# techshoww/RoMa

Hardware: AMD Instinct MI355X
Metric: image-pairs/sec at 560->864 (higher is better)
Workload: dtype fp16; 1 GPU; roma_outdoor 560->864 full coarse-to-fine symmetric match (BASELINE configs[1]; configs[2] = --pairs 8 --gpus 8); launch=eager launches, coarse_res=560, upsample_res=864, parallelism=single GPU

## Files before the change

include/roma_hip.h:

```cpp
#ifndef ROMA_HIP_H
#define ROMA_HIP_H

#include <stdint.h>

#ifdef __cplusplus
extern "C" {
#endif

#define ROMA_ABI_VERSION 5

enum { ROMA_F32 = 0, ROMA_F16 = 1, ROMA_BF16 = 2 };
enum { ROMA_NCHW = 0, ROMA_NHWC = 1 };
enum { ROMA_LC_AUTO = 0, ROMA_LC_TILE8X4 = 1, ROMA_LC_TILE8X8 = 2, ROMA_LC_ROWS8 = 3 };
enum { ROMA_E_ARG = -1, ROMA_E_DTYPE = -2, ROMA_E_SHAPE = -3, ROMA_E_ALIGN = -4, ROMA_E_UNSUPPORTED = -5 };

int roma_abi_version(void);
const char* roma_last_error(void);

int roma_local_corr(const void* f0, const void* f1, const float* flow, void* out,
                    int B, int C, int H, int W, int r, int dtype,
                    int layout, int f0_pitch, int f1_pitch, int out_layout, int out_pitch, int f1_batch_shift, int variant,
                    void* stream);

int roma_warp_bilinear(const void* src, const float* flow, void* dst,
// ... 13 lines not shown
                          void* stream);

int roma_flow_update(float* flow, float* cert, const float* cert_in, const float* delta,
                     int B, int H, int W, float sx, float sy, void* stream);

int roma_cls_to_flow_refine(const void* logits, float* flow_out, float* cert_out,
                            int B, int C, int HW, long stride_b, long stride_c, long stride_p,
                            int dtype, void* stream);

int roma_cos_kernel(const void* x, const void* y, float* K, int B, int N, int M, int D, int dtype, int x_pitch, int y_pitch,
                    int y_batch_shift, float T, float eps, float diag_add, void* stream);

int roma_chol_diag_block(float* A, int lda, long strideA, float* W, int ldw, long strideW, int nb, int B, int* info,
                         int info_base, void* stream);

int roma_chol_step(float* A, int lda, long strideA, int n, int ncols, int j, int nb, const float* W, int ldw, long strideW, float* R,
                   int ldr, long strideR, float* Wn, int ldwn, long strideWn, int* info, int info_base, int B, void* stream);

int roma_chol_subst_step(int dir, const float* W, int ldw, long strideW, const float* R, long strideRb, long strideRs, int ldr, float* T,
                         long strideTb, long strideTs, int ldt, int t_in_panel, float* X, int ldx, long strideX, int n, int m, int nb,
                         int s, int B, void* stream);

int roma_attention_fwd(const void* q, const void* k, const void* v, void* o, int B, int H, int Nq, int Nk, int head_dim, long q_sb,
                       long q_sn, long q_sh, long k_sb, long k_sn, long k_sh, long v_sb, long v_sn, long v_sh, long o_sb, long o_sn,
                       long o_sh, float scale, int dtype, void* stream);

int roma_match_finalize(const float* flow, const float* cert, const float* cert16, float* warp, float* certainty,
                        int P, int H, int W, int H16, int W16, int symmetric, void* stream);

int roma_kde_density(const float* x, float* density, int N, int down, float std, int half_mode, void* stream);

int roma_race_keys(const float* p, const long* counter, float* keys, long N, float thresh, unsigned seed, unsigned stage,
                   void* stream);

long roma_race_select_workspace(int P, long N, int k);
int roma_race_select(const float* p, const long* counter, const long* seeds, int P, long N, int k, float thresh, unsigned stage,
                     long* sel_key, long* sel_idx, void* workspace, long workspace_bytes, void* stream);

int roma_kde_density_batch(const float* x, const long* index, float* density, int P, long N, int n, int down, float std,
                           int half_mode, void* stream);

int roma_nn_argmin(const float* q, const float* r, int* idx, int NQ, int NR, void* stream);

int roma_resample_u8(const void* in, void* out, int H, int W, int C, int out_size, int axis, const int* bounds,
                     const int* coef, int ksize, void* stream);
int roma_normalize_u8(const void* in, float* out, int H, int W, const float* mean3, const float* std3, void* stream);

int roma_bias_relu_nchw(void* x, const void* bias, int B, int C, int HW, int dtype, void* stream);

int roma_bias_relu_pool2_nchw(void* x, const void* bias, void* pooled, int B, int C, int H, int W, int dtype, void* stream);

int roma_bias_relu_nhwc(void* x, const void* bias, long npix, int C, int dtype, void* stream);
int roma_bias_relu_pool2_nhwc(void* x, const void* bias, void* pooled, int B, int C, int H, int W, int dtype, void* stream);

int roma_dwconv5x5_bn_relu(const void* x, const float* w, const float* scale, const float* shift, void* y,
                           int B, int C, int H, int W, int dtype, int x_pitch, int y_pitch, void* stream);

int roma_refiner_block(const void* x, const void* w25, const float* scale, const float* shift, const void* wt,
                       const float* bias, void* y, int B, int C, int H, int W, int kpad, int dtype, int x_pitch, int y_pitch,
                       void* stream);

int roma_refiner_wide_pack(const void* wt, void* wp, int D);
int roma_refiner_wide_taps(const void* w25, void* w25p, int D);
int roma_refiner_block_wide(const void* x, const void* w25p, const float* scale, const float* shift, const void* wp,
                            const float* bias, void* y, int B, int H, int W, int D, int x_pitch, int y_pitch, int dtype,
                            void* stream);

int roma_pointwise_mfma(const void* x, const void* wt, const float* bias, void* y, long M, int C, int kpad, int dtype,
                        int x_pitch, int y_pitch, void* stream);

int roma_refiner_block_mid(const void* x, const float* w25, const float* scale, const float* shift, const void* wt,
                           const float* bias, void* y, int B, int C, int H, int W, int dtype, int x_pitch, int y_pitch,
                           void* stream);

int roma_refiner_head(const void* x, const float* wo, const float* bo, float* flow, const float* cert_in, float* cert_out,
                      float* delta_out, int B, int H, int W, int C, int pitch, int dtype, float sx, float sy, void* stream);

int roma_pointwise_small(const void* x, const float* wt, const float* bias, void* y, long M, int C, int dtype,
                         int x_pitch, int y_pitch, void* stream);

int roma_project_skinny(const void* x, const void* wt, const float* bias, void* y, long M, int K, int N, int dtype, int x_pitch,
                        int y_pitch, void* stream);

int roma_add_layernorm(void* x, int x_dtype, long x_stride, const void* y, int y_dtype, long y_stride, const float* ls,
                       const float* gamma, const float* beta, void* out, int out_dtype, long out_stride, long rows, int C,
                       float eps, void* stream);

int roma_tiny_corr_posembed(const float* f0, const float* f1, float* out, int B, int C,
                            int H0, int W0, int H1, int W1, int exact, void* stream);

int roma_jpeg_info(const void* data, long nbytes, int* info);
int roma_jpeg_entropy_decode(const void* data, long nbytes, int16_t* coef, uint16_t* qt);
int roma_jpeg_reconstruct(const int16_t* coef, const uint16_t* qt, void* planes, void* rgb, const int* info, void* stream);

long roma_ransac_workspace(int kind, int P, int N, int iters, long* offsets);
int roma_ransac_hypotheses(int kind, const double* xa, const double* xb, int P, int N, int iters, float threshold, unsigned seed,
                           int p0, void* ws, long ws_bytes, void* stream);
int roma_ransac_select(int kind, const double* xa, const double* xb, int P, int N, int iters, float threshold, int lo_iters,
                       const void* ws, long ws_bytes, double* model, unsigned char* mask, void* stream);

int roma_ransac_hypotheses_ex(int kind, const double* xa, const double* xb, int P, int N, int iters, float threshold, int scoring,
                              unsigned seed, int p0, void* ws, long ws_bytes, void* stream);
int roma_ransac_select_ex(int kind, const double* xa, const double* xb, int P, int N, int iters, float threshold, int scoring,
                          int lo_iters, const void* ws, long ws_bytes, double* model, unsigned char* mask, void* stream);
int roma_magsac_table(float* loss, float* weight);

// ... 60 lines not shown
```

roma_amd/_lib.py:

```python
from __future__ import annotations

import ctypes
import os
from ctypes import c_char_p, c_float, c_int, c_long, c_void_p

_HERE = os.path.dirname(os.path.abspath(__file__))
LIB_PATH = os.path.join(_HERE, "csrc", "libroma_hip.so")

ROMA_F32, ROMA_F16, ROMA_BF16 = 0, 1, 2
ROMA_NCHW, ROMA_NHWC = 0, 1
LC_VARIANTS = {"auto": 0, "tile8x4": 1, "tile8x8": 2, "rows8": 3}
ABI_VERSION = 5
SCORE_MSAC, SCORE_MAGSAC = 0, 1
ROMA_E_ARG, ROMA_E_DTYPE, ROMA_E_SHAPE, ROMA_E_ALIGN, ROMA_E_UNSUPPORTED = -1, -2, -3, -4, -5

SIGNATURES = {
    "roma_abi_version": [],
    "roma_last_error": [],
    "roma_local_corr": [c_void_p, c_void_p, c_void_p, c_void_p, c_int, c_int, c_int, c_int, c_int, c_int,
                        c_int, c_int, c_int, c_int, c_int, c_int, c_int, c_void_p],
    "roma_warp_bilinear": [c_void_p, c_void_p, c_void_p, c_int, c_int, c_int, c_int, c_int, c_int, c_int,
                           c_int, c_int, c_int, c_int, c_int, c_void_p],
    "roma_disp_emb": [c_void_p, c_void_p, c_void_p, c_void_p, c_int, c_int, c_int, c_int, c_float, c_int, c_int, c_int, c_void_p],
    "roma_interp_bilinear": [c_void_p, c_void_p, c_int, c_int, c_int, c_int, c_int, c_void_p],
    "roma_interp_bilinear_pair": [c_void_p, c_void_p, c_int, c_void_p, c_void_p, c_int, c_int, c_int, c_int, c_int, c_void_p],
    "roma_refiner_assemble": [c_void_p, c_void_p, c_void_p, c_void_p, c_void_p, c_int, c_int, c_int, c_int, c_int, c_int, c_int, c_int,
                              c_int, c_int, c_int, c_float, c_int, c_void_p],
    "roma_project_skinny": [c_void_p, c_void_p, c_void_p, c_void_p, c_long, c_int, c_int, c_int, c_int, c_int, c_void_p],
    "roma_flow_update": [c_void_p, c_void_p, c_void_p, c_void_p, c_int, c_int, c_int, c_float, c_float, c_void_p],
    "roma_cls_to_flow_refine": [c_void_p, c_void_p, c_void_p, c_int, c_int, c_int, c_long, c_long, c_long, c_int, c_void_p],
    "roma_cos_kernel": [c_void_p, c_void_p, c_void_p, c_int, c_int, c_int, c_int, c_int, c_int, c_int, c_int, c_float, c_float,
                        c_float, c_void_p],
    "roma_add_layernorm": [c_void_p, c_int, c_long, c_void_p, c_int, c_long, c_void_p, c_void_p, c_void_p, c_void_p, c_int, c_long,
                           c_long, c_int, c_float, c_void_p],
    "roma_attention_fwd": [c_void_p, c_void_p, c_void_p, c_void_p, c_int, c_int, c_int, c_int, c_int] + [c_long] * 12 + [c_float, c_int, c_void_p],
    "roma_chol_diag_block": [c_void_p, c_int, c_long, c_void_p, c_int, c_long, c_int, c_int, c_void_p, c_int, c_void_p],
    "roma_chol_step": [c_void_p, c_int, c_long, c_int, c_int, c_int, c_int, c_void_p, c_int, c_long, c_void_p, c_int, c_long,
                       c_void_p, c_int, c_long, c_void_p, c_int, c_int, c_void_p],
    "roma_chol_subst_step": [c_int, c_void_p, c_int, c_long, c_void_p, c_long, c_long, c_int, c_void_p, c_long, c_long, c_int, c_int,
                             c_void_p, c_int, c_long, c_int, c_int, c_int, c_int, c_int, c_void_p],
    "roma_match_finalize": [c_void_p, c_void_p, c_void_p, c_void_p, c_void_p, c_int, c_int, c_int, c_int, c_int, c_int, c_void_p],
    "roma_kde_density": [c_void_p, c_void_p, c_int, c_int, c_float, c_int, c_void_p],
    "roma_nn_argmin": [c_void_p, c_void_p, c_void_p, c_int, c_int, c_void_p],
    "roma_race_keys": [c_void_p, c_void_p, c_void_p, c_long, c_float, ctypes.c_uint, ctypes.c_uint, c_void_p],
    "roma_race_select_workspace": [c_int, c_long, c_int],
    "roma_race_select": [c_void_p, c_void_p, c_void_p, c_int, c_long, c_int, c_float, ctypes.c_uint, c_void_p, c_void_p, c_void_p, c_long,
                         c_void_p],
    "roma_kde_density_batch": [c_void_p, c_void_p, c_void_p, c_int, c_long, c_int, c_int, c_float, c_int, c_void_p],
    "roma_dwconv5x5_bn_relu": [c_void_p, c_void_p, c_void_p, c_void_p, c_void_p, c_int, c_int, c_int, c_int, c_int, c_int, c_int, c_void_p],
    "roma_resample_u8": [c_void_p, c_void_p, c_int, c_int, c_int, c_int, c_int, c_void_p, c_void_p, c_int, c_void_p],
    "roma_normalize_u8": [c_void_p, c_void_p, c_int, c_int, c_void_p, c_void_p, c_void_p],
    "roma_bias_relu_nchw": [c_void_p, c_void_p, c_int, c_int, c_int, c_int, c_void_p],
    "roma_bias_relu_pool2_nchw": [c_void_p, c_void_p, c_void_p, c_int, c_int, c_int, c_int, c_int, c_void_p],
    "roma_bias_relu_nhwc": [c_void_p, c_void_p, c_long, c_int, c_int, c_void_p],
    "roma_bias_relu_pool2_nhwc": [c_void_p, c_void_p, c_void_p, c_int, c_int, c_int, c_int, c_int, c_void_p],
    "roma_pointwise_mfma": [c_void_p, c_void_p, c_void_p, c_void_p, c_long, c_int, c_int, c_int, c_int, c_int, c_void_p],
    "roma_refiner_block": [c_void_p, c_void_p, c_void_p, c_void_p, c_void_p, c_void_p, c_void_p, c_int, c_int, c_int, c_int, c_int, c_int,
                           c_int, c_int, c_void_p],
    "roma_refiner_block_mid": [c_void_p, c_void_p, c_void_p, c_void_p, c_void_p, c_void_p, c_void_p, c_int, c_int, c_int, c_int, c_int, c_int,
                               c_int, c_void_p],
    "roma_refiner_wide_pack": [c_void_p, c_void_p, c_int],
    "roma_refiner_wide_taps": [c_void_p, c_void_p, c_int],
    "roma_jpeg_info": [c_void_p, c_long, c_void_p],
    "roma_jpeg_entropy_decode": [c_void_p, c_long, c_void_p, c_void_p],
    "roma_jpeg_reconstruct": [c_void_p, c_void_p, c_void_p, c_void_p, c_void_p, c_void_p],
    "roma_refiner_block_wide": [c_void_p, c_void_p, c_void_p, c_void_p, c_void_p, c_void_p, c_void_p, c_int, c_int, c_int, c_int, c_int, c_int,
                                c_int, c_void_p],
    "roma_refiner_head": [c_void_p, c_void_p, c_void_p, c_void_p, c_void_p, c_void_p, c_void_p, c_int, c_int, c_int, c_int, c_int, c_int,
                          c_float, c_float, c_void_p],
    "roma_pointwise_small": [c_void_p, c_void_p, c_void_p, c_void_p, c_long, c_int, c_int, c_int, c_int, c_void_p],
    "roma_tiny_corr_posembed": [c_void_p, c_void_p, c_void_p, c_int, c_int, c_int, c_int, c_int, c_int, c_int, c_void_p],
    "roma_ransac_workspace": [c_int, c_int, c_int, c_int, c_void_p],
    "roma_ransac_hypotheses": [c_int, c_void_p, c_void_p, c_int, c_int, c_int, c_float, ctypes.c_uint, c_int, c_void_p, c_long, c_void_p],
    "roma_ransac_select": [c_int, c_void_p, c_void_p, c_int, c_int, c_int, c_float, c_int, c_void_p, c_long, c_void_p, c_void_p,
                           c_void_p],
    "roma_ransac_hypotheses_ex": [c_int, c_void_p, c_void_p, c_int, c_int, c_int, c_float, c_int, ctypes.c_uint, c_int, c_void_p, c_long,
                                  c_void_p],
    "roma_ransac_select_ex": [c_int, c_void_p, c_void_p, c_int, c_int, c_int, c_float, c_int, c_int, c_void_p, c_long, c_void_p, c_void_p,
                              c_void_p],
    "roma_magsac_table": [c_void_p, c_void_p],
    "roma_essential_workspace": [c_int, c_int, c_int, c_void_p],
    "roma_essential_hypotheses": [c_void_p, c_void_p, c_void_p, c_void_p, c_int, c_int, c_int, c_float, ctypes.c_uint, c_int, c_void_p,
                                  c_long, c_void_p],
    "roma_essential_select": [c_void_p, c_void_p, c_void_p, c_void_p, c_int, c_int, c_int, c_float, c_int, c_void_p, c_long, c_void_p,
                              c_void_p, c_void_p],
    "roma_essential_hypotheses_ex": [c_void_p, c_void_p, c_void_p, c_void_p, c_int, c_int, c_int, c_float, c_int, ctypes.c_uint, c_int,
                                     c_void_p, c_long, c_void_p],
    "roma_essential_select_ex": [c_void_p, c_void_p, c_void_p, c_void_p, c_int, c_int, c_int, c_float, c_int, c_int, c_void_p, c_long,
                                 c_void_p, c_void_p, c_void_p],
    "roma_recover_pose": [c_void_p, c_void_p, c_void_p, c_void_p, c_void_p, c_void_p, c_int, c_int, c_void_p, c_void_p, c_void_p,
                          c_void_p, c_void_p],
    "roma_refine_pose": [c_void_p, c_void_p, c_void_p, c_void_p, c_void_p, c_void_p, c_void_p, c_int, c_int, ctypes.c_double, c_int,
                         c_void_p, c_void_p, c_void_p, c_void_p, c_void_p, c_void_p, c_void_p],
    "roma_refine_fundamental": [c_void_p, c_void_p, c_void_p, c_void_p, c_int, c_int, ctypes.c_double, c_int, c_void_p, c_void_p, c_void_p,
                                c_void_p, c_void_p, c_void_p],
    "roma_refine_homography": [c_void_p, c_void_p, c_void_p, c_void_p, c_int, c_int, ctypes.c_double, c_int, c_void_p, c_void_p, c_void_p,
                               c_void_p, c_void_p, c_void_p],
    "roma_triangulate": [c_void_p, c_void_p, c_void_p, c_void_p, c_void_p, c_void_p, c_void_p, c_int, c_int, c_int, c_float, c_float,
                         c_void_p, c_void_p, c_void_p, c_void_p, c_void_p, c_void_p, c_void_p],
    "roma_triangulate_nview": [c_void_p, c_void_p, c_void_p, c_long, c_void_p, c_void_p, c_void_p, c_int, c_int, c_int, c_long, c_long,
                               c_float, c_int, c_int, c_int, c_float, c_float, c_void_p, c_void_p, c_void_p, c_void_p, c_void_p, c_void_p,
                               c_void_p],
    "roma_warp_kpts": [c_void_p, c_int, c_void_p, c_void_p, c_void_p, c_void_p, c_void_p, c_int, c_int, c_int, c_int, c_int, c_int, c_int,
                       ctypes.c_double, c_void_p, c_void_p, c_void_p, c_void_p],
    "roma_dense_match_metrics": [c_void_p, c_long, c_void_p, c_void_p, c_void_p, c_void_p, c_void_p, c_int, c_int, c_int, c_int, c_int, c_int,
                                 c_int, c_int, ctypes.c_double, c_void_p, c_long, c_void_p, c_void_p, c_void_p, c_void_p, c_void_p],
    "roma_absolute_pose_workspace": [c_int, c_int, c_int, c_void_p],
    "roma_absolute_pose_hypotheses": [c_void_p, c_void_p, c_void_p, c_int, c_int, c_int, c_float, c_int, ctypes.c_uint, c_int, c_void_p,
# ... 42 lines not shown
```

roma_amd/csrc/bias_relu.hip:

```cpp
#include "common.h"

namespace roma {
namespace {

template <typename T, int VEC>
__global__ __launch_bounds__(256) void bias_relu_kernel(T* __restrict__ x, const T* __restrict__ bias, int C, int HW) {
  const int plane = blockIdx.y;
  const float bv = to_f32(bias[plane % C]);
  T* p = x + (size_t)plane * HW;
  const int nvec = HW / VEC;
  for (int i = blockIdx.x * 256 + threadIdx.x; i < nvec; i += gridDim.x * 256) {
    if constexpr (VEC == 8) {
      u32x4 v = reinterpret_cast<u32x4*>(p)[i];
      float f[8];
      unpack16<T>(v, f);
#pragma unroll
      for (int e = 0; e < 8; ++e) f[e] = fmaxf(f[e] + bv, 0.f);
      reinterpret_cast<u32x4*>(p)[i] = pack16<T>(f);
    } else {
#pragma unroll
      for (int e = 0; e < VEC; ++e) p[i * VEC + e] = from_f32<T>(fmaxf(to_f32(p[i * VEC + e]) + bv, 0.f));
    }
  }
}
// ... 51 lines not shown
      o[e] = from_f32<T>(fmaxf(fmaxf(a[2 * e], a[2 * e + 1]), fmaxf(b[2 * e], b[2 * e + 1])));
  }
}

template <typename T>
__global__ __launch_bounds__(256) void bias_relu_nhwc_kernel(T* __restrict__ x, const T* __restrict__ bias, long npack, int cpack) {
  constexpr int E = ElemTraits<T>::kPer16B;
  for (long i = (long)blockIdx.x * 256 + threadIdx.x; i < npack; i += (long)gridDim.x * 256) {
    float f[E], bb[E];
    unpack16<T>(reinterpret_cast<const u32x4*>(x)[i], f);
    unpack16<T>(reinterpret_cast<const u32x4*>(bias)[i % cpack], bb);
#pragma unroll
    for (int e = 0; e < E; ++e) f[e] = fmaxf(f[e] + bb[e], 0.f);
    reinterpret_cast<u32x4*>(x)[i] = pack16<T>(f);
  }
}

template <typename T>
__global__ __launch_bounds__(256) void bias_relu_pool_nhwc_kernel(T* __restrict__ x, const T* __restrict__ bias, T* __restrict__ pooled,
                                                                 int B, int H, int W, int cpack) {
  constexpr int E = ElemTraits<T>::kPer16B;
  const int Ho = H / 2, Wo = W / 2;
  const long n = (long)B * Ho * Wo * cpack;
  u32x4* xv = reinterpret_cast<u32x4*>(x);
  for (long i = (long)blockIdx.x * 256 + threadIdx.x; i < n; i += (long)gridDim.x * 256) {
    const int cp = (int)(i % cpack);
    long r = i / cpack;
    const int xo = (int)(r % Wo);
    r /= Wo;
    const int yo = (int)(r % Ho), b = (int)(r / Ho);
    float bb[E], m[E];
    unpack16<T>(reinterpret_cast<const u32x4*>(bias)[cp], bb);
#pragma unroll
    for (int e = 0; e < E; ++e) m[e] = 0.f;
#pragma unroll
    for (int dy = 0; dy < 2; ++dy)
#pragma unroll
      for (int dx = 0; dx < 2; ++dx) {
        const long idx = (((long)b * H + 2 * yo + dy) * W + 2 * xo + dx) * cpack + cp;
        float f[E];
        unpack16<T>(xv[idx], f);
#pragma unroll
        for (int e = 0; e < E; ++e) { f[e] = fmaxf(f[e] + bb[e], 0.f); }
        const u32x4 pk = pack16<T>(f);
        xv[idx] = pk;
        unpack16<T>(pk, f);
#pragma unroll
        for (int e = 0; e < E; ++e) m[e] = fmaxf(m[e], f[e]);
      }
    reinterpret_cast<u32x4*>(pooled)[i] = pack16<T>(m);
  }
}

}
}

using namespace roma;

extern "C" int roma_bias_relu_nhwc(void* x, const void* bias, long npix, int C, int dtype, void* stream) {
  ROMA_REQUIRE(x && bias, ROMA_E_ARG, "roma_bias_relu_nhwc: null pointer");
  const int e16 = dtype == ROMA_F32 ? 4 : 8;
  ROMA_REQUIRE(npix > 0 && C > 0 && C % e16 == 0 && aligned16(x) && aligned16(bias), ROMA_E_ALIGN,
               "roma_bias_relu_nhwc: C = %d must be a multiple of %d and the buffers 16-byte aligned", C, e16);
  hipStream_t s = static_cast<hipStream_t>(stream);
  const long npack = npix * (C / e16);
  const unsigned grid = (unsigned)((npack + 255) / 256 < 65536 ? (npack + 255) / 256 : 65536);
  switch (dtype) {
    case ROMA_F32: hipLaunchKernelGGL((bias_relu_nhwc_kernel<float>), dim3(grid), dim3(256), 0, s, (float*)x, (const float*)bias, npack, C / e16); break;
    case ROMA_F16: hipLaunchKernelGGL((bias_relu_nhwc_kernel<half_t>), dim3(grid), dim3(256), 0, s, (half_t*)x, (const half_t*)bias, npack, C / e16); break;
    case ROMA_BF16: hipLaunchKernelGGL((bias_relu_nhwc_kernel<bf16_t>), dim3(grid), dim3(256), 0, s, (bf16_t*)x, (const bf16_t*)bias, npack, C / e16); break;
    default: ROMA_REQUIRE(false, ROMA_E_DTYPE, "roma_bias_relu_nhwc: dtype %d", dtype);
  }
  ROMA_CHECK_LAUNCH();
}

extern "C" int roma_bias_relu_pool2_nhwc(void* x, const void* bias, void* pooled, int B, int C, int H, int W, int dtype, void* stream) {
  ROMA_REQUIRE(x && bias && pooled, ROMA_E_ARG, "roma_bias_relu_pool2_nhwc: null pointer");
  const int e16 = dtype == ROMA_F32 ? 4 : 8;
  ROMA_REQUIRE(B > 0 && H > 0 && W > 0 && H % 2 == 0 && W % 2 == 0, ROMA_E_SHAPE, "roma_bias_relu_pool2_nhwc: bad shape B=%d H=%d W=%d (even H, W)", B, H, W);
  ROMA_REQUIRE(C > 0 && C % e16 == 0 && aligned16(x) && aligned16(bias) && aligned16(pooled), ROMA_E_ALIGN,
               "roma_bias_relu_pool2_nhwc: C = %d must be a multiple of %d and the buffers 16-byte aligned", C, e16);
  hipStream_t s = static_cast<hipStream_t>(stream);
  const long n = (long)B * (H / 2) * (W / 2) * (C / e16);
  const unsigned grid = (unsigned)((n + 255) / 256 < 65536 ? (n + 255) / 256 : 65536);
  switch (dtype) {
    case ROMA_F32: hipLaunchKernelGGL((bias_relu_pool_nhwc_kernel<float>), dim3(grid), dim3(256), 0, s, (float*)x, (const float*)bias, (float*)pooled, B, H, W, C / e16); break;
    case ROMA_F16: hipLaunchKernelGGL((bias_relu_pool_nhwc_kernel<half_t>), dim3(grid), dim3(256), 0, s, (half_t*)x, (const half_t*)bias, (half_t*)pooled, B, H, W, C / e16); break;
    case ROMA_BF16: hipLaunchKernelGGL((bias_relu_pool_nhwc_kernel<bf16_t>), dim3(grid), dim3(256), 0, s, (bf16_t*)x, (const bf16_t*)bias, (bf16_t*)pooled, B, H, W, C / e16); break;
    default: ROMA_REQUIRE(false, ROMA_E_DTYPE, "roma_bias_relu_pool2_nhwc: dtype %d", dtype);
  }
  ROMA_CHECK_LAUNCH();
}

extern "C" int roma_bias_relu_pool2_nchw(void* x, const void* bias, void* pooled, int B, int C, int H, int W, int dtype, void* stream) {
  ROMA_REQUIRE(x && bias && pooled, ROMA_E_ARG, "roma_bias_relu_pool2_nchw: null pointer");
  ROMA_REQUIRE(B > 0 && C > 0 && H > 0 && W > 0 && (long)B * C <= 65535 && H % 2 == 0 && W % 2 == 0, ROMA_E_SHAPE,
               "roma_bias_relu_pool2_nchw: bad shape B=%d C=%d H=%d W=%d (even H, W; B*C <= 65535)", B, C, H, W);
  ROMA_REQUIRE(dtype >= ROMA_F32 && dtype <= ROMA_BF16, ROMA_E_DTYPE, "roma_bias_relu_pool2_nchw: dtype %d", dtype);
  hipStream_t s = static_cast<hipStream_t>(stream);
  const int planes = B * C;
  auto gridx = [&](int vec) { const int n = ((H / 2) * (W / vec) + 255) / 256; return n < 64 ? n : 64; };
  const bool v8 = dtype != ROMA_F32 && W % 8 == 0 && aligned16(x);
#define ROMA_BRP(T, V) hipLaunchKernelGGL((bias_relu_pool_kernel<T, V>), dim3(gridx(V), planes), dim3(256), 0, s, (T*)x, (const T*)bias, (T*)pooled, C, H, W)
  if (dtype == ROMA_F32) ROMA_BRP(float, 2);
  else if (dtype == ROMA_F16) { if (v8) ROMA_BRP(half_t, 8); else ROMA_BRP(half_t, 2); }
  else { if (v8) ROMA_BRP(bf16_t, 8); else ROMA_BRP(bf16_t, 2); }
#undef ROMA_BRP
  ROMA_CHECK_LAUNCH();
}

extern "C" int roma_bias_relu_nchw(void* x, const void* bias, int B, int C, int HW, int dtype, void* stream) {
  ROMA_REQUIRE(x && bias, ROMA_E_ARG, "roma_bias_relu_nchw: null pointer");
  ROMA_REQUIRE(B > 0 && C > 0 && HW > 0 && (long)B * C <= 65535, ROMA_E_SHAPE, "roma_bias_relu_nchw: bad shape B=%d C=%d HW=%d", B, C, HW);
  hipStream_t s = static_cast<hipStream_t>(stream);
  const int planes = B * C;
  auto gridx = [&](int vec) { const int n = (HW / vec + 255) / 256; return n < 64 ? n : 64; };
  if (dtype == ROMA_F32) {
    if (HW % 4 == 0 && aligned16(x)) hipLaunchKernelGGL((bias_relu_kernel_f32<4>), dim3(gridx(4), planes), dim3(256), 0, s, (float*)x, (const float*)bias, C, HW);
    else hipLaunchKernelGGL((bias_relu_kernel_f32<1>), dim3(gridx(1), planes), dim3(256), 0, s, (float*)x, (const float*)bias, C, HW);
  } else if (dtype == ROMA_F16 || dtype == ROMA_BF16) {
    const bool v8 = HW % 8 == 0 && aligned16(x);
    if (dtype == ROMA_F16) {
      if (v8) hipLaunchKernelGGL((bias_relu_kernel<half_t, 8>), dim3(gridx(8), planes), dim3(256), 0, s, (half_t*)x, (const half_t*)bias, C, HW);
      else hipLaunchKernelGGL((bias_relu_kernel<half_t, 1>), dim3(gridx(1), planes), dim3(256), 0, s, (half_t*)x, (const half_t*)bias, C, HW);
    } else {
      if (v8) hipLaunchKernelGGL((bias_relu_kernel<bf16_t, 8>), dim3(gridx(8), planes), dim3(256), 0, s, (bf16_t*)x, (const bf16_t*)bias, C, HW);
      else hipLaunchKernelGGL((bias_relu_kernel<bf16_t, 1>), dim3(gridx(1), planes), dim3(256), 0, s, (bf16_t*)x, (const bf16_t*)bias, C, HW);
    }
  } else {
    ROMA_REQUIRE(false, ROMA_E_DTYPE, "roma_bias_relu_nchw: dtype %d", dtype);
  }
  ROMA_CHECK_LAUNCH();
}
```

roma_amd/encoders.py:

```python
from __future__ import annotations

from typing import Optional

import torch
import torch.nn as nn
import torch.nn.functional as F

from . import ops

from .transformer import DinoViT

VGG19_CFG = [64, 64, "M", 128, 128, "M", 256, 256, 256, 256, "M", 512, 512, 512, 512, "M", 512, 512, 512, 512, "M"]


def _ver(t):
    return 0 if t.is_inference() else t._version


class VGG19(nn.Module):

    def __init__(self):
        super().__init__()
        layers, c = [], 3
        for v in VGG19_CFG:
            if v == "M":
                layers.append(nn.MaxPool2d(2, 2))
            else:
                layers += [nn.Conv2d(c, v, 3, padding=1), nn.BatchNorm2d(v), nn.ReLU(inplace=True)]
                c = v
        self.layers = nn.ModuleList(layers[:40])
        self._folded = None

    def fold(self, dtype, nhwc=False):
        key = (dtype, nhwc, self.layers[0].weight.device, tuple(_ver(p) for p in self.parameters()))
        if self._folded is not None and self._folded[0] == key:
            return self._folded[1]
        plan = []
        i = 0
        while i < len(self.layers):
            m = self.layers[i]
            if isinstance(m, nn.MaxPool2d):
                plan.append(None)
                i += 1
                continue
            bn = self.layers[i + 1]
            s = bn.weight.float() / torch.sqrt(bn.running_var.float() + bn.eps)
            w = (m.weight.float() * s[:, None, None, None]).to(dtype).contiguous(memory_format=torch.channels_last if nhwc else torch.contiguous_format)
            b = ((m.bias.float() - bn.running_mean.float()) * s + bn.bias.float()).to(dtype)
            plan.append((w, b))
            i += 3
        self._folded = (key, plan)
        return plan

    @torch.no_grad()
    def forward(self, x, dtype=torch.float16):
        feats, scale = {}, 1
        nhwc = torch.backends.cudnn.benchmark and x.is_cuda
        x = x.to(dtype).contiguous(memory_format=torch.channels_last if nhwc else torch.contiguous_format)
        plan = self.fold(dtype, nhwc)
        for i, step in enumerate(plan):
            if step is None:
                continue
            pooled_next = i + 1 < len(plan) and plan[i + 1] is None
            x = F.conv2d(x, step[0], None, padding=1)
            if not pooled_next:
                x = ops.bias_relu_(x, step[1])
                continue
            feats[scale] = x
            last = i + 2 >= len(plan)
            if last or x.shape[-1] % 2 or x.shape[-2] % 2:
                ops.bias_relu_(x, step[1])
                x = None if last else F.max_pool2d(x, 2, 2)
            else:
                x = ops.bias_relu_pool2_(x, step[1])
            scale *= 2
        return feats


def enable_miopen_find():
    import os
    if os.environ.get("ROMA_MIOPEN_FIND", "1") != "0":
        torch.backends.cudnn.benchmark = True


class CNNandDinov2(nn.Module):
    def __init__(self, dinov2: Optional[DinoViT] = None, amp_dtype=torch.float16):
        super().__init__()
        enable_miopen_find()
        self.cnn = VGG19()
        self.amp_dtype = amp_dtype
        self.dinov2_vitl14 = [dinov2 if dinov2 is not None else DinoViT()]

    def train(self, mode: bool = True):
        return self.cnn.train(mode)

    def _vit(self, device):
        master = self.dinov2_vitl14[0]
        key = (str(device), self.amp_dtype, tuple(_ver(p) for p in master.parameters()))
        cache = self.__dict__.setdefault("_vit_cache", {})
        hit = cache.get(key)
        if hit is None:
            import copy
            cache.clear()
            if self.amp_dtype == torch.float32 and next(master.parameters()).device == device:
                hit = master.eval()
            else:
                with torch.inference_mode(False), torch.no_grad():
                    hit = copy.deepcopy(master).to(device=device, dtype=self.amp_dtype).eval()
            cache[key] = hit
        return hit

    @torch.no_grad()
    def vit_features(self, x):
        B, C, H, W = x.shape
        t = self._vit(x.device).patch_tokens(x.to(self.amp_dtype))
        return t.reshape(B, H // 14, W // 14, -1).permute(0, 3, 1, 2)

    @torch.no_grad()
    def forward(self, x, upsample=False):
        pyr = self.cnn(x, self.amp_dtype)
        if not upsample:
            pyr[16] = self.vit_features(x)
        return pyr
# ... 1 lines not shown
```

roma_amd/ops.py:

```python
from __future__ import annotations

import math
from typing import Optional

import torch

from . import _lib
from ._lib import ROMA_BF16, ROMA_F16, ROMA_F32, ROMA_NCHW, ROMA_NHWC, check

_DT = {torch.float32: ROMA_F32, torch.float16: ROMA_F16, torch.bfloat16: ROMA_BF16}


class KernelTimer:

    def __init__(self):
        self.enabled = False
        self.bracket_overhead_s = 0.0
        self.records = []

    def start(self):
        self.records.clear()
        torch.cuda.synchronize()
        pairs = []
        for _ in range(32):
# ... 527 lines not shown
    return out


def normalize_u8(img, mean, std):
    import ctypes
    _need_gpu(img)
    H, W, C = img.shape
    assert C == 3 and img.dtype == torch.uint8 and img.is_contiguous()
    out = torch.empty((3, H, W), dtype=torch.float32, device=img.device)
    m = (ctypes.c_float * 3)(*mean)
    s = (ctypes.c_float * 3)(*std)
    check(_lib.load().roma_normalize_u8(_p(img), _p(out), H, W, ctypes.cast(m, ctypes.c_void_p), ctypes.cast(s, ctypes.c_void_p), _stream()),
          "roma_normalize_u8")
    return out


def _is_nhwc(x):
    return x.dim() == 4 and x.shape[1] > 1 and x.stride(1) == 1 and x.is_contiguous(memory_format=torch.channels_last)


def bias_relu_(x, bias):
    _need_gpu(x, bias)
    B, C, H, W = x.shape
    assert bias.dtype == x.dtype and bias.numel() == C and bias.is_contiguous()
    if _is_nhwc(x):
        check(_lib.load().roma_bias_relu_nhwc(_p(x), _p(bias), B * H * W, C, _dt(x), _stream()), "roma_bias_relu_nhwc")
        return x
    assert x.is_contiguous()
    step = max(1, 65535 // C)
    for b0 in range(0, B, step):
        xb = x[b0:b0 + step]
        check(_lib.load().roma_bias_relu_nchw(_p(xb), _p(bias), xb.shape[0], C, H * W, _dt(x), _stream()), "roma_bias_relu_nchw")
    return x


def bias_relu_pool2_(x, bias):
    _need_gpu(x, bias)
    B, C, H, W = x.shape
    assert bias.dtype == x.dtype and bias.numel() == C and bias.is_contiguous() and H % 2 == 0 and W % 2 == 0
    if _is_nhwc(x):
        out = torch.empty((B, H // 2, W // 2, C), dtype=x.dtype, device=x.device).permute(0, 3, 1, 2)
        check(_lib.load().roma_bias_relu_pool2_nhwc(_p(x), _p(bias), _p(out), B, C, H, W, _dt(x), _stream()), "roma_bias_relu_pool2_nhwc")
        return out
    assert x.is_contiguous()
    out = torch.empty((B, C, H // 2, W // 2), dtype=x.dtype, device=x.device)
    step = max(1, 65535 // C)
    for b0 in range(0, B, step):
        xb = x[b0:b0 + step]
        check(_lib.load().roma_bias_relu_pool2_nchw(_p(xb), _p(bias), _p(out[b0:b0 + step]), xb.shape[0], C, H, W, _dt(x), _stream()),
              "roma_bias_relu_pool2_nchw")
    return out


def pointwise_mfma(rows, wt, bias, C, out=None):
    _need_gpu(rows, wt, bias, out)
    M, pitch = rows.shape
    kpad = wt.shape[0]
    assert rows.is_contiguous() and wt.is_contiguous() and wt.dtype == rows.dtype and bias.numel() == kpad and bias.dtype == torch.float32
    if out is None:
        out = torch.empty_like(rows)
    assert out.shape == rows.shape and out.is_contiguous()
    check(_lib.load().roma_pointwise_mfma(_p(rows), _p(wt), _p(bias), _p(out), M, C, kpad, _dt(rows), pitch, pitch, _stream()),
          "roma_pointwise_mfma")
    return out


def project_skinny_pack(wt_in_out, bias):
    K, N = wt_in_out.shape
    Np = (N + 15) // 16 * 16
    wt = torch.zeros((Np, K), dtype=wt_in_out.dtype, device=wt_in_out.device)
    wt[:N] = wt_in_out.t()
    b = torch.zeros(Np, dtype=torch.float32, device=wt_in_out.device)
    b[:N] = bias.float()
    return wt, b


def project_skinny(rows, wt, bias, N, out):
    _need_gpu(rows, wt, bias, out)
    M, K = rows.shape
    if rows.stride(1) != 1 or out.stride(1) != 1 or out.shape[0] != M or out.shape[1] < N or out.dtype != rows.dtype or wt.dtype != rows.dtype:
        raise ValueError("project_skinny: rows (M,K) and out (M,>=N) must be unit-stride rows of one 16-bit dtype")
    if not wt.is_contiguous() or wt.shape[1] != K or wt.shape[0] < N or bias.dtype != torch.float32 or bias.numel() != wt.shape[0]:
        raise ValueError("project_skinny: wt / bias are not what project_skinny_pack returns for these rows")
    check(_lib.load().roma_project_skinny(_p(rows), _p(wt), _p(bias), _p(out), M, K, N, _dt(rows), rows.stride(0), out.stride(0), _stream()),
          "roma_project_skinny")
    return out


def refiner_wide_pack(wt_out_in):
    w = wt_out_in.detach().to("cpu").contiguous()
    assert w.dim() == 2 and w.shape[0] == w.shape[1] and w.element_size() == 2
    out = torch.empty_like(w)
    check(_lib.load().roma_refiner_wide_pack(w.data_ptr(), out.data_ptr(), w.shape[0]), "roma_refiner_wide_pack")
    return out.to(wt_out_in.device)


def refiner_wide_taps(w25, dtype=torch.float16):
    D = w25.shape[1]
    w = w25.detach().to("cpu").to(dtype).contiguous()
    assert w.shape == (25, D) and w.element_size() == 2
    out = torch.empty((D // 32, 5, 4, 2, 6, 4, 2), dtype=dtype)
    check(_lib.load().roma_refiner_wide_taps(w.data_ptr(), out.data_ptr(), D), "roma_refiner_wide_taps")
    return out.to(w25.device)


def refiner_block_wide(x_nhwc, w25p, scale, shift, wp, bias, out=None):
# ... 106 lines not shown
```

Before: 61.12 image-pairs/s.

## Use tuned CK conv3x3 kernels with fused bias-ReLU for fp16 NHWC VGG layers

```diff
diff --git a/include/roma_hip.h b/include/roma_hip.h
--- a/include/roma_hip.h
+++ b/include/roma_hip.h
@@ -89,6 +89,12 @@
 
 int roma_bias_relu_nhwc(void* x, const void* bias, long npix, int C, int dtype, void* stream);
 int roma_bias_relu_pool2_nhwc(void* x, const void* bias, void* pooled, int B, int C, int H, int W, int dtype, void* stream);
+
+int roma_maxpool2_nhwc(const void* x, void* pooled, int B, int C, int H, int W, int dtype, void* stream);
+
+int roma_conv3x3_bias_relu(const void* x, const void* w, const void* bias, void* y, int B, int Cin, int Cout, int H, int W, int dtype,
+                           int x_pitch, int y_pitch, int instance, void* stream);
+int roma_conv3x3_bias_relu_instances(int index, char* name, int cap);
 
 int roma_dwconv5x5_bn_relu(const void* x, const float* w, const float* scale, const float* shift, void* y,
                            int B, int C, int H, int W, int dtype, int x_pitch, int y_pitch, void* stream);
diff --git a/roma_amd/_lib.py b/roma_amd/_lib.py
--- a/roma_amd/_lib.py
+++ b/roma_amd/_lib.py
@@ -54,6 +54,9 @@
     "roma_bias_relu_pool2_nchw": [c_void_p, c_void_p, c_void_p, c_int, c_int, c_int, c_int, c_int, c_void_p],
     "roma_bias_relu_nhwc": [c_void_p, c_void_p, c_long, c_int, c_int, c_void_p],
     "roma_bias_relu_pool2_nhwc": [c_void_p, c_void_p, c_void_p, c_int, c_int, c_int, c_int, c_int, c_void_p],
+    "roma_maxpool2_nhwc": [c_void_p, c_void_p, c_int, c_int, c_int, c_int, c_int, c_void_p],
+    "roma_conv3x3_bias_relu": [c_void_p, c_void_p, c_void_p, c_void_p, c_int, c_int, c_int, c_int, c_int, c_int, c_int, c_int, c_int, c_void_p],
+    "roma_conv3x3_bias_relu_instances": [c_int, c_char_p, c_int],
     "roma_pointwise_mfma": [c_void_p, c_void_p, c_void_p, c_void_p, c_long, c_int, c_int, c_int, c_int, c_int, c_void_p],
     "roma_refiner_block": [c_void_p, c_void_p, c_void_p, c_void_p, c_void_p, c_void_p, c_void_p, c_int, c_int, c_int, c_int, c_int, c_int,
                            c_int, c_int, c_void_p],
diff --git a/roma_amd/csrc/bias_relu.hip b/roma_amd/csrc/bias_relu.hip
--- a/roma_amd/csrc/bias_relu.hip
+++ b/roma_amd/csrc/bias_relu.hip
@@ -127,6 +127,31 @@
   }
 }
 
+template <typename T>
+__global__ __launch_bounds__(256) void maxpool2_nhwc_kernel(const T* __restrict__ x, T* __restrict__ pooled, int B, int H, int W, int cpack) {
+  constexpr int E = ElemTraits<T>::kPer16B;
+  const int Ho = H / 2, Wo = W / 2;
+  const long n = (long)B * Ho * Wo * cpack;
+  const u32x4* xv = reinterpret_cast<const u32x4*>(x);
+  for (long i = (long)blockIdx.x * 256 + threadIdx.x; i < n; i += (long)gridDim.x * 256) {
+    const int cp = (int)(i % cpack);
+    long r = i / cpack;
+    const int xo = (int)(r % Wo);
+    r /= Wo;
+    const int yo = (int)(r % Ho), b = (int)(r / Ho);
+    const long idx = (((long)b * H + 2 * yo) * W + 2 * xo) * cpack + cp;
+    float m[E], f[E];
+    unpack16<T>(xv[idx], m);
+#pragma unroll
+    for (int k = 1; k < 4; ++k) {
+      unpack16<T>(xv[idx + ((k >> 1) * (long)W + (k & 1)) * cpack], f);
+#pragma unroll
+      for (int e = 0; e < E; ++e) m[e] = fmaxf(m[e], f[e]);
+    }
+    reinterpret_cast<u32x4*>(pooled)[i] = pack16<T>(m);
+  }
+}
+
 }
 }
 
@@ -163,6 +188,24 @@
     case ROMA_F16: hipLaunchKernelGGL((bias_relu_pool_nhwc_kernel<half_t>), dim3(grid), dim3(256), 0, s, (half_t*)x, (const half_t*)bias, (half_t*)pooled, B, H, W, C / e16); break;
     case ROMA_BF16: hipLaunchKernelGGL((bias_relu_pool_nhwc_kernel<bf16_t>), dim3(grid), dim3(256), 0, s, (bf16_t*)x, (const bf16_t*)bias, (bf16_t*)pooled, B, H, W, C / e16); break;
     default: ROMA_REQUIRE(false, ROMA_E_DTYPE, "roma_bias_relu_pool2_nhwc: dtype %d", dtype);
+  }
+  ROMA_CHECK_LAUNCH();
+}
+
+extern "C" int roma_maxpool2_nhwc(const void* x, void* pooled, int B, int C, int H, int W, int dtype, void* stream) {
+  ROMA_REQUIRE(x && pooled, ROMA_E_ARG, "roma_maxpool2_nhwc: null pointer");
+  ROMA_REQUIRE(dtype >= ROMA_F32 && dtype <= ROMA_BF16, ROMA_E_DTYPE, "roma_maxpool2_nhwc: dtype %d", dtype);
+  const int e16 = dtype == ROMA_F32 ? 4 : 8;
+  ROMA_REQUIRE(B > 0 && H > 0 && W > 0 && H % 2 == 0 && W % 2 == 0, ROMA_E_SHAPE, "roma_maxpool2_nhwc: bad shape B=%d H=%d W=%d (even H, W)", B, H, W);
+  ROMA_REQUIRE(C > 0 && C % e16 == 0 && aligned16(x) && aligned16(pooled), ROMA_E_ALIGN,
+               "roma_maxpool2_nhwc: C = %d must be a multiple of %d and the buffers 16-byte aligned", C, e16);
+  hipStream_t s = static_cast<hipStream_t>(stream);
+  const long n = (long)B * (H / 2) * (W / 2) * (C / e16);
+  const unsigned grid = (unsigned)((n + 255) / 256 < 65536 ? (n + 255) / 256 : 65536);
+  switch (dtype) {
+    case ROMA_F32: hipLaunchKernelGGL((maxpool2_nhwc_kernel<float>), dim3(grid), dim3(256), 0, s, (const float*)x, (float*)pooled, B, H, W, C / e16); break;
+    case ROMA_F16: hipLaunchKernelGGL((maxpool2_nhwc_kernel<half_t>), dim3(grid), dim3(256), 0, s, (const half_t*)x, (half_t*)pooled, B, H, W, C / e16); break;
+    default: hipLaunchKernelGGL((maxpool2_nhwc_kernel<bf16_t>), dim3(grid), dim3(256), 0, s, (const bf16_t*)x, (bf16_t*)pooled, B, H, W, C / e16); break;
   }
   ROMA_CHECK_LAUNCH();
 }
diff --git a/roma_amd/csrc/vgg_conv.hip b/roma_amd/csrc/vgg_conv.hip
--- /dev/null
+++ b/roma_amd/csrc/vgg_conv.hip
@@ -0,0 +1,57 @@
+#include <climits>
+#include <cstring>
+
+#include "common.h"
+#include "vgg_conv_instances.h"
+
+using namespace roma;
+
+namespace {
+
+vggconv::InstanceFn find_instance(int index) {
+  const vggconv::InstanceList lists[] = {vggconv::instances_a(), vggconv::instances_b(), vggconv::instances_c()};
+  for (const auto& l : lists) {
+    if (index < l.n) return l.fn[index];
+    index -= l.n;
+  }
+  return nullptr;
+}
+
+int instance_count() { return vggconv::instances_a().n + vggconv::instances_b().n + vggconv::instances_c().n; }
+
+}
+
+extern "C" int roma_conv3x3_bias_relu_instances(int index, char* name, int cap) {
+  const int n = instance_count();
+  if (!name) return n;
+  ROMA_REQUIRE(index >= 0 && index < n && cap > 0, ROMA_E_ARG, "roma_conv3x3_bias_relu_instances: index %d of %d, cap %d", index, n, cap);
+  std::string s;
+  find_instance(index)(vggconv::ConvArgs{}, vggconv::kName, &s);
+  std::strncpy(name, s.c_str(), (size_t)cap - 1);
+  name[cap - 1] = 0;
+  return n;
+}
+
+extern "C" int roma_conv3x3_bias_relu(const void* x, const void* w, const void* bias, void* y, int B, int Cin, int Cout, int H, int W,
+                                      int dtype, int x_pitch, int y_pitch, int instance, void* stream) {
+  ROMA_REQUIRE(x && w && bias && y, ROMA_E_ARG, "roma_conv3x3_bias_relu: null pointer");
+  ROMA_REQUIRE(dtype == ROMA_F16, dtype == ROMA_F32 || dtype == ROMA_BF16 ? ROMA_E_UNSUPPORTED : ROMA_E_DTYPE,
+               "roma_conv3x3_bias_relu: dtype %d (fp16 only)", dtype);
+  ROMA_REQUIRE(B > 0 && Cin > 0 && Cout > 0 && H > 0 && W > 0 && x_pitch >= Cin && y_pitch >= Cout, ROMA_E_SHAPE,
+               "roma_conv3x3_bias_relu: bad shape B=%d Cin=%d Cout=%d H=%d W=%d x_pitch=%d y_pitch=%d", B, Cin, Cout, H, W, x_pitch, y_pitch);
+  ROMA_REQUIRE((long)B * H * W * (x_pitch > y_pitch ? x_pitch : y_pitch) <= INT_MAX && (long)Cout * 9 * Cin <= INT_MAX, ROMA_E_SHAPE,
+               "roma_conv3x3_bias_relu: a map of B=%d H=%d W=%d with pitch %d / %d exceeds 2^31 - 1 elements", B, H, W, x_pitch, y_pitch);
+  ROMA_REQUIRE(Cin % 8 == 0 && Cout % 8 == 0 && x_pitch % 8 == 0 && y_pitch % 8 == 0 && aligned16(x) && aligned16(w) && aligned16(bias) &&
+                   aligned16(y), ROMA_E_ALIGN,
+               "roma_conv3x3_bias_relu: Cin = %d, Cout = %d and the pitches %d / %d must be multiples of 8 and the buffers 16-byte aligned",
+               Cin, Cout, x_pitch, y_pitch);
+  const vggconv::InstanceFn fn = instance >= 0 ? find_instance(instance) : nullptr;
+  ROMA_REQUIRE(fn, ROMA_E_ARG, "roma_conv3x3_bias_relu: instance %d of %d", instance, instance_count());
+  const vggconv::ConvArgs a{x, w, bias, y, B, Cin, Cout, H, W, x_pitch, y_pitch, static_cast<hipStream_t>(stream)};
+  std::string what;
+  const int rc = fn(a, vggconv::kRun, &what);
+  ROMA_REQUIRE(rc != ROMA_E_UNSUPPORTED, ROMA_E_UNSUPPORTED,
+               "roma_conv3x3_bias_relu: instance %d does not support B=%d Cin=%d Cout=%d H=%d W=%d on this device", instance, B, Cin, Cout, H, W);
+  ROMA_REQUIRE(rc == 0, rc, "roma_conv3x3_bias_relu: launch failed: %s", what.c_str());
+  ROMA_CHECK_LAUNCH();
+}
diff --git a/roma_amd/csrc/vgg_conv_a.hip b/roma_amd/csrc/vgg_conv_a.hip
--- /dev/null
+++ b/roma_amd/csrc/vgg_conv_a.hip
@@ -0,0 +1,18 @@
+#include "vgg_conv_instances.h"
+#include "ck/tensor_operation/gpu/device/impl/device_grouped_conv_fwd_multiple_abd_xdl_cshuffle.hpp"
+
+namespace roma {
+namespace vggconv {
+
+InstanceList instances_a() {
+  static const InstanceFn fn[] = {
+      run_instance<ROMA_CONV_V1(256, 128, 64, 32, 2, 1, 32, 8)>,
+      run_instance<ROMA_CONV_V1(256, 256, 128, 32, 4, 2, 32, 8)>,
+      run_instance<ROMA_CONV_V1(256, 128, 128, 32, 2, 2, 32, 8)>,
+      run_instance<ROMA_CONV_V1(128, 128, 128, 32, 4, 2, 16, 8)>,
+  };
+  return {fn, (int)(sizeof(fn) / sizeof(fn[0]))};
+}
+
+}
+}
diff --git a/roma_amd/csrc/vgg_conv_b.hip b/roma_amd/csrc/vgg_conv_b.hip
--- /dev/null
+++ b/roma_amd/csrc/vgg_conv_b.hip
@@ -0,0 +1,18 @@
+#include "vgg_conv_instances.h"
+#include "ck/tensor_operation/gpu/device/impl/device_grouped_conv_fwd_multiple_abd_xdl_cshuffle.hpp"
+
+namespace roma {
+namespace vggconv {
+
+InstanceList instances_b() {
+  static const InstanceFn fn[] = {
+      run_instance<ROMA_CONV_V1(128, 64, 128, 32, 2, 2, 16, 8)>,
+      run_instance<ROMA_CONV_V1(256, 128, 256, 32, 2, 4, 32, 8)>,
+      run_instance<ROMA_CONV_V1(128, 128, 64, 32, 2, 2, 32, 4)>,
+      run_instance<ROMA_CONV_V1(256, 64, 128, 32, 1, 2, 32, 8)>,
+  };
+  return {fn, (int)(sizeof(fn) / sizeof(fn[0]))};
+}
+
+}
+}
diff --git a/roma_amd/csrc/vgg_conv_c.hip b/roma_amd/csrc/vgg_conv_c.hip
--- /dev/null
+++ b/roma_amd/csrc/vgg_conv_c.hip
@@ -0,0 +1,16 @@
+#include "vgg_conv_instances.h"
+#include "ck/tensor_operation/gpu/device/impl/device_grouped_conv_fwd_multiple_abd_xdl_cshuffle_v3.hpp"
+
+namespace roma {
+namespace vggconv {
+
+InstanceList instances_c() {
+  static const InstanceFn fn[] = {
+      run_instance<ROMA_CONV_V3(128, 128, 64, 8, 8, 0, Intrawave, v4)>,
+      run_instance<ROMA_CONV_V3(128, 128, 64, 16, 4, 1, Interwave, v1)>,
+  };
+  return {fn, (int)(sizeof(fn) / sizeof(fn[0]))};
+}
+
+}
+}
diff --git a/roma_amd/csrc/vgg_conv_instances.h b/roma_amd/csrc/vgg_conv_instances.h
--- /dev/null
+++ b/roma_amd/csrc/vgg_conv_instances.h
@@ -0,0 +1,104 @@
+#pragma once
+#include <array>
+#include <exception>
+#include <string>
+
+#include <hip/hip_runtime.h>
+
+#include "error.h"
+
+#include "ck/ck.hpp"
+#include "ck/stream_config.hpp"
+#include "ck/tensor_operation/gpu/device/convolution_forward_specialization.hpp"
+#include "ck/tensor_operation/gpu/device/gemm_specialization.hpp"
+#include "ck/tensor_operation/gpu/device/tensor_layout.hpp"
+#include "ck/tensor_operation/gpu/element/element_wise_operation.hpp"
+
+namespace roma {
+namespace vggconv {
+
+struct BiasReluRound {
+  static constexpr const char* name = "BiasReluRound";
+  template <typename E, typename C, typename D>
+  __host__ __device__ constexpr void operator()(E& e, const C& c, const D& d) const {
+    const ck::half_t r = ck::type_convert<ck::half_t>(c);
+    e = ck::type_convert<E>(fmaxf(ck::type_convert<float>(r) + ck::type_convert<float>(d), 0.f));
+  }
+};
+
+struct ConvArgs {
+  const void* x;
+  const void* w;
+  const void* bias;
+  void* y;
+  int B, Cin, Cout, H, W, x_pitch, y_pitch;
+  hipStream_t stream;
+};
+
+enum Mode { kName, kCheck, kRun };
+
+using InstanceFn = int (*)(const ConvArgs& a, Mode mode, std::string* name);
+
+struct InstanceList {
+  const InstanceFn* fn;
+  int n;
+};
+InstanceList instances_a();
+InstanceList instances_b();
+InstanceList instances_c();
+
+using F16 = ck::half_t;
+using F32 = float;
+template <ck::index_t... Is>
+using S = ck::Sequence<Is...>;
+using NHWGC = ck::tensor_layout::convolution::NHWGC;
+using GKYXC = ck::tensor_layout::convolution::GKYXC;
+using NHWGK = ck::tensor_layout::convolution::NHWGK;
+using PassThrough = ck::tensor_operation::element_wise::PassThrough;
+constexpr auto kConvDefault = ck::tensor_operation::device::ConvolutionForwardSpecialization::Default;
+constexpr auto kMNKPadding = ck::tensor_operation::device::GemmSpecialization::MNKPadding;
+
+template <typename Op>
+int run_instance(const ConvArgs& a, Mode mode, std::string* name) {
+  Op op;
+  if (mode == kName) {
+    *name = op.GetTypeString();
+    return 0;
+  }
+  using Arr = std::array<ck::index_t, 5>;
+  const int B = a.B, C = a.Cin, K = a.Cout, H = a.H, W = a.W, xp = a.x_pitch, yp = a.y_pitch;
+  const Arr x_len{1, B, C, H, W}, x_str{C, H * W * xp, 1, W * xp, xp};
+  const Arr w_len{1, K, C, 3, 3}, w_str{K * 9 * C, 9 * C, 1, 3 * C, C};
+  const Arr y_len{1, B, K, H, W}, y_str{K, H * W * yp, 1, W * yp, yp};
+  const Arr b_str{K, 0, 1, 0, 0};
+  const std::array<ck::index_t, 2> one{1, 1};
+  try {
+    auto arg = op.MakeArgument(a.x, a.w, std::array<const void*, 1>{a.bias}, a.y, x_len, x_str, w_len, w_str,
+                               std::array<Arr, 1>{y_len}, std::array<Arr, 1>{b_str}, y_len, y_str, one, one, one, one,
+                               PassThrough{}, PassThrough{}, BiasReluRound{});
+    if (!op.IsSupportedArgument(arg)) return ROMA_E_UNSUPPORTED;
+    if (mode == kCheck) return 0;
+    op.MakeInvoker().Run(arg, StreamConfig{a.stream, false});
+  } catch (const std::exception& e) {
+    *name = e.what();
+    const int rc = (int)hipGetLastError();
+    return rc ? rc : (int)hipErrorUnknown;
+  }
+  return 0;
+}
+
+#define ROMA_CONV_V1(BLK, M, N, K, MX, NX, CM, CN)                                                                                  \
+  ck::tensor_operation::device::DeviceGroupedConvFwdMultipleABD_Xdl_CShuffle<                                                       \
+      2, NHWGC, GKYXC, ck::Tuple<NHWGK>, NHWGK, F16, F16, F32, F16, ck::Tuple<F16>, F16, PassThrough, PassThrough, BiasReluRound,   \
+      kConvDefault, kMNKPadding, 1, BLK, M, N, K, 8, 8, 32, 32, MX, NX, S<4, BLK / 4, 1>, S<1, 0, 2>, S<1, 0, 2>, 2, 8, 8, 1,        \
+      S<4, BLK / 4, 1>, S<1, 0, 2>, S<1, 0, 2>, 2, 8, 8, 1, 1, 1, S<1, CM, 1, CN>, 8>
+
+#define ROMA_CONV_V3(M, N, K, K1, K0, PAD, SCHED, VER)                                                                              \
+  ck::tensor_operation::device::DeviceGroupedConvFwdMultipleABD_Xdl_CShuffle_V3<                                                    \
+      2, NHWGC, GKYXC, ck::Tuple<NHWGK>, NHWGK, F16, F16, F32, F16, ck::Tuple<F16>, F16, PassThrough, PassThrough, BiasReluRound,   \
+      kConvDefault, kMNKPadding, 256, M, N, K, K1, K1, 32, 32, 2, 2, S<K0, 256 / K0, 1>, S<1, 0, 2>, S<1, 0, 2>, 2, 8, 8, PAD,      \
+      S<K0, 256 / K0, 1>, S<1, 0, 2>, S<1, 0, 2>, 2, 8, 8, PAD, 1, 1, S<1, 32, 1, 8>, 8, ck::BlockGemmPipelineScheduler::SCHED,     \
+      ck::BlockGemmPipelineVersion::VER>
+
+}
+}
diff --git a/roma_amd/encoders.py b/roma_amd/encoders.py
--- a/roma_amd/encoders.py
+++ b/roma_amd/encoders.py
@@ -17,6 +17,26 @@
     return 0 if t.is_inference() else t._version
 
 
+VGG_CONV_TABLE = {
+    (64, 64): ((627200, 1492992, 6),),
+    (64, 128): ((156800, 156800, 2), (373248, 373248, 1)),
+    (128, 128): ((156800, 156800, 8), (373248, 373248, 1)),
+    (128, 256): ((39200, 39200, 2), (93312, 93312, 1)),
+    (256, 256): ((93312, 93312, 8),),
+    (256, 512): ((9800, 23328, 8),),
+    (512, 512): ((9800, 23328, 8),),
+}
+
+
+def vgg_conv_impl(dtype, nhwc, Cin, Cout, B, H, W):
+    if dtype != torch.float16 or not nhwc:
+        return "library"
+    for lo, hi, instance in VGG_CONV_TABLE.get((Cin, Cout), ()):
+        if lo <= B * H * W <= hi:
+            return instance
+    return "library"
+
+
 class VGG19(nn.Module):
 
     def __init__(self):
@@ -30,6 +50,7 @@
                 c = v
         self.layers = nn.ModuleList(layers[:40])
         self._folded = None
+        self.conv_impl = vgg_conv_impl
 
     def fold(self, dtype, nhwc=False):
         key = (dtype, nhwc, self.layers[0].weight.device, tuple(_ver(p) for p in self.parameters()))
@@ -62,13 +83,22 @@
             if step is None:
                 continue
             pooled_next = i + 1 < len(plan) and plan[i + 1] is None
+            last = i + 2 >= len(plan)
+            even = x.shape[-1] % 2 == 0 and x.shape[-2] % 2 == 0
+            impl = self.conv_impl(dtype, nhwc, x.shape[1], step[0].shape[0], x.shape[0], x.shape[2], x.shape[3])
+            if impl != "library":
+                x = ops.conv3x3_bias_relu(x, step[0], step[1], impl)
+                if pooled_next:
+                    feats[scale] = x
+                    x = None if last else ops.maxpool2_nhwc(x) if even else F.max_pool2d(x, 2, 2)
+                    scale *= 2
+                continue
             x = F.conv2d(x, step[0], None, padding=1)
             if not pooled_next:
                 x = ops.bias_relu_(x, step[1])
                 continue
             feats[scale] = x
-            last = i + 2 >= len(plan)
-            if last or x.shape[-1] % 2 or x.shape[-2] % 2:
+            if last or not even:
                 ops.bias_relu_(x, step[1])
                 x = None if last else F.max_pool2d(x, 2, 2)
             else:
diff --git a/roma_amd/ops.py b/roma_amd/ops.py
--- a/roma_amd/ops.py
+++ b/roma_amd/ops.py
@@ -603,6 +603,45 @@
     return out
 
 
+def maxpool2_nhwc(x):
+    _need_gpu(x)
+    B, C, H, W = x.shape
+    assert _is_nhwc(x) and H % 2 == 0 and W % 2 == 0
+    out = torch.empty((B, H // 2, W // 2, C), dtype=x.dtype, device=x.device).permute(0, 3, 1, 2)
+    check(_lib.load().roma_maxpool2_nhwc(_p(x), _p(out), B, C, H, W, _dt(x), _stream()), "roma_maxpool2_nhwc")
+    return out
+
+
+def conv3x3_instances():
+    import ctypes
+    lib = _lib.load()
+    buf = ctypes.create_string_buffer(256)
+    names = []
+    for i in range(lib.roma_conv3x3_bias_relu_instances(0, None, 0)):
+        check(min(0, lib.roma_conv3x3_bias_relu_instances(i, buf, len(buf))), "roma_conv3x3_bias_relu_instances")
+        names.append(buf.value.decode())
+    return names
+
+
+def conv3x3_bias_relu(x, w, bias, instance, out=None):
+    _need_gpu(x, w, bias, out)
+    B, Cin, H, W = x.shape
+    Cout = w.shape[0]
+    assert w.shape == (Cout, Cin, 3, 3) and w.dtype == x.dtype == bias.dtype and bias.numel() == Cout and bias.is_contiguous()
+    assert w.permute(0, 2, 3, 1).is_contiguous(), "w must be channels-last (KYXC in memory)"
+    if out is None:
+        out = torch.empty((B, H, W, Cout), dtype=x.dtype, device=x.device).permute(0, 3, 1, 2)
+    assert out.shape == (B, Cout, H, W) and out.dtype == x.dtype
+
+    def pitch(t):
+        sb, sc, sh, sw = t.stride()
+        assert sc == 1 and sh == t.shape[3] * sw and sb == t.shape[2] * sh, "channels-last pixel rows expected"
+        return sw
+    check(_lib.load().roma_conv3x3_bias_relu(_p(x), _p(w), _p(bias), _p(out), B, Cin, Cout, H, W, _dt(x), pitch(x), pitch(out),
+                                             int(instance), _stream()), "roma_conv3x3_bias_relu")
+    return out
+
+
 def pointwise_mfma(rows, wt, bias, C, out=None):
     _need_gpu(rows, wt, bias, out)
     M, pitch = rows.shape
```

New measurement: 62.21 image-pairs/s, median of 6. 1.02x the previous value.
